# staghado/vit.cpp

Hardware: AMD Instinct MI355X
Metric: images/sec ViT-B/16 224^2 bs=256 per GPU (forward, synthetic, HBM-resident inputs) (higher is better)
Workload: dtype bf16

## Files before the change

vit.cpp_amd/csrc/engine.cpp:

```cpp
#include <hip/hip_runtime.h>
#include <stdio.h>
#include <stdlib.h>
#include <string.h>

#include <algorithm>
#include <map>
#include <memory>
#include <mutex>
#include <new>
#include <string>
#include <tuple>
#include <vector>

#include "kernels.h"
#include "model_file.h"

using namespace vitx;

#define HIP_TRY(expr)                                                                                      \
    do {                                                                                                   \
        hipError_t e__ = (expr);                                                                           \
        if (e__ != hipSuccess) { set_error("%s failed: %s (%s:%d)", #expr, hipGetErrorString(e__), __FILE__, __LINE__); return VITX_ERR_HIP; } \
    } while (0)

// ... 43 lines not shown
        void *pe_w = nullptr, *head_w = nullptr;
        QuantW head_q;
        std::vector<LayerW> layers;
        size_t weight_bytes = 0;
        ~WeightSet() {
            int cur = -1; (void)hipGetDevice(&cur);
            (void)hipSetDevice(device); for (void *p : allocs) (void)hipFree(p);
            if (cur >= 0 && cur != device) (void)hipSetDevice(cur);
        }
    };
    std::shared_ptr<WeightSet> wset;
    bool weights_shared = false;
    float *cls = nullptr, *pos = nullptr, *pe_b = nullptr, *norm_w = nullptr, *norm_b = nullptr, *head_b = nullptr;
    void *pe_w = nullptr, *head_w = nullptr;
    QuantW head_q;
    std::vector<LayerW> layers;
    bool quant_on_device = true;
    int q4_fused_rows = 0;
    size_t weight_bytes = 0;
    bool prec_attn = false;
    bool cls_tail = true;
    bool ln_fuse = true;
    unsigned ln_epoch = 0;
    unsigned ln_timeout = 20000;
    int ln_test = 0;
    int call_limit = 0;
    unsigned *ln_fb_host = nullptr;
    unsigned long long ln_fb_base = 0;
    int ln_fb_forwards = 0;
    bool ln_fuse_disabled = false;
    int ln_cool_left = 0, ln_cool_len = 256;
    struct Slice {
        int cap = 0;
        float *X = nullptr;
        void *U = nullptr;
        void *U2 = nullptr;
        unsigned long long *ln_sync = nullptr;
        unsigned *ln_todo = nullptr;
        int ln_blocks = 0;
        void *QKV = nullptr;
        long qkv_lo_off = 0;
        void *Hbuf = nullptr;
        float *Xc = nullptr;
        void *Z = nullptr;
        void *Wq[W_PER_LAYER] = {nullptr, nullptr, nullptr, nullptr};
        void *Wq_head = nullptr;
        float *logits = nullptr;
        hipStream_t stream = nullptr;
        hipEvent_t done = nullptr;
        Tuning tune;
    };
    int nslices = 1;
    std::vector<Slice> slices;
    hipEvent_t fork = nullptr;
    std::vector<hipStream_t> probed_streams;
    int stream_retries = 0;
    hipEvent_t probe_a = nullptr, probe_b = nullptr;
    float *img = nullptr;
    float *probs = nullptr;
    float *logits_all = nullptr;
// ... 173 lines not shown
    c->D = hp.hidden_size; c->L = hp.num_hidden_layers; c->H = hp.num_attention_heads; c->C = hp.num_classes; c->P = hp.patch_size; c->S = hp.img_size;
    c->Cin = m->in_chans; c->R = m->in_chans == 1 ? VITX_VITSTR_SEQ_LEN : 1;
    c->g = c->S / c->P; c->N = c->g * c->g + 1; c->Kpe = c->Cin * c->P * c->P; c->Kpe_pad = round_up(c->Kpe, 64);
    if (c->N < c->R) { set_error("vitx_ctx_create: a ViTSTR head reads %d tokens, this model has %d (img_size %d, patch_size %d)", c->R, c->N, c->S, c->P); return VITX_ERR_UNSUPPORTED; }
    c->tm = gemm_tile_m(); c->tn = gemm_tile_n();
    c->C_pad = round_up(c->C, c->tn);
    if (!attention_supports(c->N, c->D, c->H)) {
        set_error("vitx_ctx_create: attention needs a head_dim that is a multiple of 8 up to 128 (this model: %d) and at least one token (%d tokens, img_size %d, patch_size %d)", c->D / c->H, c->N, c->S, c->P);
        return VITX_ERR_UNSUPPORTED;
    }
    if (!layernorm_supports(c->D)) { set_error("vitx_ctx_create: hidden_size %d has no LayerNorm instantiation (64, 128, 192, 256, 320, 384, 448, 512, 576, 640, 768, 896, 1024, 1152, 1280, 1408, 1536, 1664, 2048)", c->D); return VITX_ERR_UNSUPPORTED; }
    c->tune = tuning_for_device(device);
    if (!c->tune) { set_error("vitx_ctx_create: kernel bring-up on device %d failed: %s", device, hipGetErrorString(hipGetLastError())); return VITX_ERR_HIP; }
    c->split_first = opt.split_first;
    c->prec_attn = dtype == VITX_F16 && c->D == c->H * 64 && !opt.f16_fast_attention;
    c->quant_on_device = !opt.quant_on_host;
    c->cls_tail = !opt.last_layer_all_rows && c->R == 1 && attention_cls_supports(c->N, c->D, c->H);
    c->q4_fused_rows = opt.q4_fused_rows;
    c->graphs_on = opt.graph != 0;
    if (opt.ln_test) {
        if ((opt.ln_test & (int32_t)0xffff0000) != (int32_t)VITX_LN_TEST_KEY) { set_error("vitx_ctx_create_ex: ln_test is a test-only switch (it needs its key: include/vitx.h)"); return VITX_ERR_ARG; }
        c->ln_test = opt.ln_test & 0xffff;
        if (c->ln_test & ~7) { set_error("vitx_ctx_create_ex: ln_test mode %d has bits outside 1 | 2 | 4", c->ln_test); return VITX_ERR_ARG; }
        if ((c->ln_test & 3) == 3) c->ln_timeout = 5000;
    }
    c->ln_fuse = !opt.no_ln_fusion && !opt.graph;
#ifdef VITX_LAB
    if (const char *e = getenv("VITX_SKIP")) c->skip = atoi(e);
    if (const char *e = getenv("VITX_SPLIT")) c->split_first = atoi(e);
#endif
    HIP_TRY(hipStreamCreateWithFlags(&c->stream, hipStreamNonBlocking));

    const int D = c->D, tn = c->tn;
    int rc;
    auto T = [&](const std::string &n) { return m->find(n); };
    static std::mutex wreg_mu;
    static std::map<std::tuple<uint64_t, int, int, int>, std::weak_ptr<vitx_ctx::WeightSet>> wreg;
    const auto wkey = std::make_tuple(m->uid, device, dtype, c->quant_on_device ? 1 : 0);
    std::unique_lock<std::mutex> wlock(wreg_mu);
    for (auto it = wreg.begin(); it != wreg.end();) it = it->second.expired() ? wreg.erase(it) : std::next(it);
    if (auto have = wreg[wkey].lock()) {
        c->wset = have; c->weights_shared = true;
    } else {
        c->wset = std::make_shared<vitx_ctx::WeightSet>();
        c->wset->device = device;
    }
    if (!c->weights_shared) {
// ... 35 lines not shown

    int ns = opt.streams > 0 ? opt.streams : 2;
    if (ns < 1) ns = 1;
    if (ns > 4) ns = 4;
    if (max_batch < 8 * ns) ns = 1;
    c->nslices = ns;
    c->slices.resize(ns);
    const size_t hcols = std::max<size_t>((size_t)4 * D, (size_t)c->Kpe_pad);
    {
        const size_t row_bytes = std::max<size_t>(hcols * 2, (size_t)3 * D * 2 * (c->prec_attn ? 2 : 1));
        const size_t rows = (size_t)0xf0000000u / row_bytes / 256 * 256;
        const long per_slice = (long)(rows / c->N);
        if (per_slice < 1) { set_error("vitx_ctx_create: a single image exceeds the kernels' 32-bit buffer window (%d tokens x %d)", c->N, D); return VITX_ERR_UNSUPPORTED; }
        c->call_limit = (int)std::min<long>((long)max_batch, per_slice);
    }
    for (int i = 0; i < ns; ++i) {
        vitx_ctx::Slice &sl = c->slices[i];
        sl.cap = std::min(max_batch, c->call_limit);
        const size_t Mpad = (size_t)round_up(sl.cap * c->N, c->tm), Bpad = (size_t)round_up(sl.cap * c->R, c->tm);
        if ((rc = c->dmalloc((void **)&sl.X, Mpad * D * 4, true))) return rc;
        if ((rc = c->dmalloc(&sl.U, Mpad * D * 2, true))) return rc;
        if ((rc = c->dmalloc(&sl.U2, Mpad * D * 2, true))) return rc;
        if (D % 256 == 0 && D / 256 <= 4) {
            if ((rc = c->dmalloc((void **)&sl.ln_sync, (Mpad / 256) * (size_t)(D / 256) * 256 * 2 * sizeof(unsigned long long), true))) return rc;
            if ((rc = c->dmalloc((void **)&sl.ln_todo, (Mpad / 256 + 1) * sizeof(unsigned), true))) return rc;
            sl.ln_blocks = (int)(Mpad / 256);
        }
        if ((rc = c->dmalloc(&sl.QKV, Mpad * 3 * D * 2 * (c->prec_attn ? 2 : 1), true))) return rc;
        sl.qkv_lo_off = c->prec_attn ? (long)(Mpad * 3 * D) : 0;
        if ((rc = c->dmalloc(&sl.Hbuf, Mpad * hcols * 2, true))) return rc;
        if ((rc = c->dmalloc(&sl.Z, Bpad * D * 2, true))) return rc;
        if (c->cls_tail && (rc = c->dmalloc((void **)&sl.Xc, Bpad * D * 4, true))) return rc;
        if ((rc = c->dmalloc((void **)&sl.logits, Bpad * c->C_pad * 4, true))) return rc;
        for (int k = 0; k < W_PER_LAYER; ++k) {
            size_t need = 0;
            for (const LayerW &w : c->layers) if (w.q[k].blocks) need = std::max(need, (size_t)w.q[k].n_pad * w.q[k].K * 2);
            if (need && (rc = c->dmalloc(&sl.Wq[k], need, false))) return rc;
        }
        if (c->head_q.blocks && (rc = c->dmalloc(&sl.Wq_head, (size_t)c->head_q.n_pad * c->head_q.K * 2, false))) return rc;
        sl.tune = *c->tune;
#ifdef VITX_LAB
        if (const char *e = getenv("VITX_SLICE_CU")) { if (ns > 1 && atoi(e) > 0) sl.tune.n_cu = atoi(e); }
#endif
        if (ns > 1 && i > 0) {
            int least = 0, greatest = 0;
            HIP_TRY(hipDeviceGetStreamPriorityRange(&least, &greatest));
            HIP_TRY(hipStreamCreateWithPriority(&sl.stream, hipStreamNonBlocking, greatest));
            HIP_TRY(hipEventCreateWithFlags(&sl.done, hipEventDisableTiming));
// ... 52 lines not shown
    auto fused_ok = [&](const QuantW &q, int rows) { return q.blocks && q.type == T_Q4_0 && rows <= c->q4_fused_rows && rows % 128 == 0 && q.n_pad % 128 == 0 && q.K % 64 == 0; };
    auto expand = [&](const QuantW *const *qs, void *const *dst, int count) -> int {
        bool done[W_PER_LAYER] = {false, false, false, false};
        for (int k = 0; k < count; ++k) {
            if (done[k] || !qs[k]) continue;
            DequantJob jobs[4]; int nj = 0; double bytes = 0;
            for (int m = k; m < count; ++m) {
                if (done[m] || !qs[m] || qs[m]->type != qs[k]->type) continue;
                jobs[nj++] = DequantJob{qs[m]->blocks, qs[m]->scales, dst[m], qs[m]->N, qs[m]->n_pad, qs[m]->K / 32};
                bytes += (double)qs[m]->N * qs[m]->K / 32 * type_block_bytes(qs[m]->type) + (double)qs[m]->n_pad * qs[m]->K * eb;
                done[m] = true;
            }
            ProfScope ps(c, st, PC_DEQUANT, 0, bytes);
            HIP_TRY(launch_dequant(dt, qs[k]->type, jobs, nj, st));
        }
        return VITX_OK;
    };
#ifdef VITX_LAB
    const int skip = c->skip;
#else
    constexpr int skip = 0;
#endif
    bool fuse = false;
    if (c->ln_fuse && sl.ln_sync) {
        GemmArgs probe{}; probe.M = M; probe.N = D; probe.N_pad = round_up(D, tn); probe.K = D; probe.lda = D; probe.ldw = D; probe.ldo = D;
        hipStreamCaptureStatus cs = hipStreamCaptureStatusNone;
        if (hipStreamIsCapturing(st, &cs) != hipSuccess) { (void)hipGetLastError(); cs = hipStreamCaptureStatusActive; }
        GemmArgs probe2 = probe; probe2.K = 4 * D; probe2.lda = 4 * D; probe2.ldw = 4 * D;
        fuse = cs == hipStreamCaptureStatusNone && gemm_ln_fusable(tn_, probe) && gemm_ln_fusable(tn_, probe2);
    }
    auto resid_gemm_ln = [&](int pc, const void *A, const void *W, const float *bias, int K, const QuantW *fq, const float *lw, const float *lb, void *ln_out, GemmLn *pend) -> int {
        int rc2;
        pend->todo = nullptr;
        if (fuse && lw && !fq) {
            GemmLn ln{};
            ln.w = lw; ln.b = lb; ln.x = sl.X; ln.out = ln_out; ln.eps = c->hp.eps; ln.sync = sl.ln_sync; ln.todo = sl.ln_todo; ln.fallbacks = sl.ln_todo + sl.ln_blocks;
            if (++c->ln_epoch == 0) c->ln_epoch = 1;
            ln.epoch = c->ln_epoch; ln.timeout = c->ln_timeout; ln.test = c->ln_test;
            if ((rc2 = gemm(c, tn_, st, pc, EPI_BIAS_RESID, A, W, bias, sl.X, nullptr, M, M, D, round_up(D, tn), K, K, K, D, 0, 4, nullptr, &ln, nullptr, 0, M_real))) return rc2;
            *pend = ln;
            return VITX_OK;
        }
        if ((rc2 = gemm(c, tn_, st, pc, EPI_BIAS_RESID, A, W, bias, sl.X, nullptr, M, M_real, D, round_up(D, tn), K, K, K, D, 0, 4, fq))) return rc2;
        if (lw) {
            ProfScope ps(c, st, PC_LAYERNORM, 0, (double)M_real * D * (4 + eb));
            if (!(skip & 2)) HIP_TRY(launch_layernorm(dt, sl.X, D, lw, lb, ln_out, D, M_real, D, c->hp.eps, st));
        }
        return VITX_OK;
    };
    GemmLn fix_u{}, fix_u2{};
    const bool tail = c->cls_tail && c->trace_ids.empty();
    const int Mc = round_up(n, tm);
    for (int il = 0; il < c->L; ++il) {
        const LayerW &w = c->layers[il];
        const bool tail_now = tail && il + 1 == c->L;
        const void *Wl[W_PER_LAYER] = {w.qkv_w, w.proj_w, w.fc1_w, w.fc2_w};
        const QuantW *Fl[W_PER_LAYER] = {nullptr, nullptr, nullptr, nullptr};
        {
            const QuantW *todo[W_PER_LAYER] = {nullptr, nullptr, nullptr, nullptr};
            bool any = false;
            for (int k = 0; k < W_PER_LAYER; ++k) {
// ... 88 lines not shown
        if (fused_ok(c->head_q, round_up(nR, tm))) head_f = &c->head_q;
        else { const QuantW *todo[1] = {&c->head_q}; void *dst[1] = {sl.Wq_head}; if ((rc = expand(todo, dst, 1))) return rc; head_w = sl.Wq_head; }
    }
    if ((rc = gemm(c, tn_, st, PC_GEMM_HEAD, EPI_BIAS_F32, sl.Z, head_w, c->head_b, lg, nullptr, round_up(nR, tm), nR, c->C, c->C_pad, D, D, D, ldl, 0, 4, head_f))) return rc;
    {
        ProfScope ps(c, st, PC_SOFTMAX, 0, (double)nR * c->C * 8);
        HIP_TRY(launch_softmax(dt, lg, (float *)d_probs, nR, c->C, ldl, st));
    }
    if (fuse && c->ln_fb_host) HIP_TRY(hipMemcpyAsync(c->ln_fb_host + (&sl - &c->slices[0]), sl.ln_todo + sl.ln_blocks, sizeof(unsigned), hipMemcpyDeviceToHost, st));
    return VITX_OK;
}

static double gemm_round_cost(long rows, int N, int K, int n_cu) {
    const long ntm = (rows + 255) / 256, ntn = (N + 255) / 256, tiles = ntm * ntn, rounds = tiles / n_cu, rem = tiles % n_cu;
    const double slots = K / 32.0, t_tile = slots * 0.98 + 3.5, t_half = slots * 0.6 + 3.0;
    if (rounds >= 1 && rem > 0 && rem <= n_cu * 6 / 10) {
        const long m_main = rounds * n_cu / ntn, half_tiles = ((ntm - m_main) * 2) * ntn;
        return rounds * t_tile + (double)((half_tiles + n_cu - 1) / n_cu) * t_half;
    }
    if (tiles < 128) return (double)(((rows + 127) / 128 * ntn + n_cu - 1) / n_cu) * t_half;
    return (double)((tiles + n_cu - 1) / n_cu) * t_tile;
}
static double gemm_round_cost_ln(long rows, int N, int K, int n_cu) {
    const long ntm = (rows + 255) / 256, ntn = N / 256;
    const int grid = gemm_ln_grid(n_cu, (int)(ntm * 256), N);
    const long most = ((ntm + 7) / 8) * ntn, wgx = grid / 8;
    return (double)((most + wgx - 1) / wgx) * (K / 32.0 * 0.98 + 3.5 + 2.0);
}
static void split_batch(const vitx_ctx *c, int n, int ns, int *m) {
    const int base = n / ns, extra = n % ns;
    for (int i = 0; i < ns; ++i) m[i] = base + (i < extra ? 1 : 0);
    if (c->split_first > 0 && ns == 2 && c->split_first < n) { m[0] = c->split_first; m[1] = n - c->split_first; return; }
    if (ns != 2) return;
    const int n_cu = c->tune->n_cu;
    const int D = c->D;
    const bool ln = c->ln_fuse && c->slices[0].ln_sync;
    if (ln) {
        const int ntn = D / 256, per_xcd = std::max(n_cu / 8, ntn) / ntn;
        const int s1 = (int)((long)8 * per_xcd * 256 / c->N);
        if (s1 >= n / 4 && s1 <= n / 2 && (long)s1 * c->N / 256 * ntn >= 128) { m[0] = s1; m[1] = n - s1; return; }
    }
    auto layer = [&](int imgs) {
        const long rows = (long)imgs * c->N;
        const bool fl = ln && ((rows + 255) / 256) * (D / 256) >= 128;
        return gemm_round_cost(rows, 3 * D, D, n_cu) + gemm_round_cost(rows, 4 * D, D, n_cu) +
               (fl ? gemm_round_cost_ln(rows, D, D, n_cu) + gemm_round_cost_ln(rows, D, 4 * D, n_cu) : gemm_round_cost(rows, D, D, n_cu) + gemm_round_cost(rows, D, 4 * D, n_cu));
    };
    double best = layer(m[0]) + layer(m[1]);
    for (int s1 = std::max(8, n / 4); s1 <= n / 2; ++s1) {
        const double cost = layer(s1) + layer(n - s1);
        if (cost < best * 0.97) { best = cost; m[0] = s1; m[1] = n - s1; }
    }
}

static int forward_graph(vitx_ctx *c, hipStream_t st, const void *d_imgs, int n, void *d_probs, void *d_logits, bool *done) {
    *done = false;
    for (auto &ge : c->graphs)
        if (ge.imgs == d_imgs && ge.n == n && ge.probs == d_probs && ge.logits == d_logits) {
            if (hipGraphLaunch(ge.exec, st) == hipSuccess) { *done = true; return VITX_OK; }
// ... 249 lines not shown
    g.M = M; g.M_real = M_real; g.N = N; g.N_pad = n_pad; g.K = K; g.lda = K; g.ldw = K; g.ldo = N; g.tpi = tpi;
    g.hilo_off = epi == EPI_BIAS_HILO ? (long)M * N : 0;
    hipError_t e = launch_gemm(t, dtype, epi, g, (hipStream_t)stream);
    if (e == hipErrorInvalidValue) { set_error("vitx_op_gemm: kernel %d cannot tile M %d N %d K %d", kernel, M, N, K); return VITX_ERR_UNSUPPORTED; }
    if (e != hipSuccess) { set_error("vitx_op_gemm: %s", hipGetErrorString(e)); return VITX_ERR_HIP; }
    return VITX_OK;
}
int vitx_op_gemm_ex(int dtype, int epi, int kernel, const void *a, const void *w, const void *bias, void *out, const void *pos, int M, int M_real, int N, int K, int tpi, void *stream) {
    return op_gemm_impl(dtype, epi, kernel, a, w, bias, out, pos, M, M_real, N, round_up(N, 256), K, tpi, stream);
}
int vitx_op_gemm(int dtype, int epi, const void *a, const void *w, const void *bias, void *out, int M, int N, int K, void *stream) {
    if (epi < 0 || epi > 3 || N % 64) { set_error("vitx_op_gemm: epi 0..3, N %% 64 == 0"); return VITX_ERR_ARG; }
    return op_gemm_impl(dtype, epi, 0, a, w, bias, out, nullptr, M, M, N, round_up(N, gemm_tile_n()), K, 0, stream);
}
int vitx_op_gemm_ln(int dtype, const void *a, const void *w, const void *bias, void *x, const void *ln_w, const void *ln_b, void *y, int M, int N, int K, float eps,
                    int test, int timeout_us, int *fallbacks, void *stream) {
    if (!a || !w || !bias || !x || !ln_w || !ln_b || !y || M <= 0 || timeout_us < 0) { set_error("vitx_op_gemm_ln: invalid argument"); return VITX_ERR_ARG; }
    const Tuning *t0 = tuning_for_device(-1);
    if (!t0) { set_error("vitx_op_gemm_ln: kernel bring-up failed"); return VITX_ERR_HIP; }
    GemmArgs g{};
    g.A = a; g.W = w; g.bias = (const float *)bias; g.out = x; g.M = M; g.M_real = M; g.N = N; g.N_pad = N; g.K = K; g.lda = K; g.ldw = K; g.ldo = N;
    if (!gemm_ln_fusable(*t0, g)) { set_error("vitx_op_gemm_ln: M %d N %d K %d does not take the LayerNorm-fusing kernel (M %% 256, N in {256,512,768,1024}, >= 128 tiles, K %% 128)", M, N, K); return VITX_ERR_UNSUPPORTED; }
    static unsigned epoch = 0x40000000u;
    const size_t nb = (size_t)M / 256, sync_bytes = nb * (N / 256) * 256 * 2 * sizeof(unsigned long long);
    unsigned long long *sync = nullptr; unsigned *todo = nullptr;
    HIP_TRY(hipMalloc((void **)&sync, sync_bytes));
    if (hipMalloc((void **)&todo, (nb + 1) * 4) != hipSuccess) { (void)hipFree(sync); return VITX_ERR_NOMEM; }
    int rc = VITX_OK;
    hipStream_t st = (hipStream_t)stream;
    GemmLn ln{};
    ln.w = (const float *)ln_w; ln.b = (const float *)ln_b; ln.out = y; ln.eps = eps; ln.sync = sync; ln.todo = todo; ln.fallbacks = todo + nb;
    ln.epoch = ++epoch; ln.timeout = (unsigned)timeout_us * 100u; ln.test = test;
    g.ln = &ln;
    hipError_t e = hipMemsetAsync(sync, 0, sync_bytes, st);
    if (e == hipSuccess) e = hipMemsetAsync(todo, 0, (nb + 1) * 4, st);
    if (e == hipSuccess) e = launch_gemm(*t0, dtype, EPI_BIAS_RESID, g, st);
    if (e == hipSuccess) e = launch_layernorm_fixup(dtype, (const float *)x, ln.w, ln.b, y, M, N, eps, todo, ln.epoch, st);
    if (e == hipSuccess) e = hipStreamSynchronize(st);
    unsigned fb = 0;
    if (e == hipSuccess) e = hipMemcpy(&fb, todo + nb, 4, hipMemcpyDeviceToHost);
    if (e != hipSuccess) { set_error("vitx_op_gemm_ln: %s", hipGetErrorString(e)); rc = VITX_ERR_HIP; }
    if (fallbacks) *fallbacks = (int)fb;
    (void)hipFree(sync); (void)hipFree(todo);
    return rc;
}
int vitx_op_dequant(int dtype, int qtype, const void *blocks, const void *scales, void *out, int N, int n_pad, int K, void *stream) {
    if (!blocks || !out || N <= 0 || n_pad < N || K <= 0 || K % 32 || (dtype != VITX_F16 && dtype != VITX_BF16)) { set_error("vitx_op_dequant: invalid argument"); return VITX_ERR_ARG; }
    DequantJob j{blocks, scales, out, N, n_pad, K / 32};
    hipError_t e = launch_dequant(dtype, qtype, &j, 1, (hipStream_t)stream);
    if (e != hipSuccess) { set_error("vitx_op_dequant: %s", hipGetErrorString(e)); return e == hipErrorInvalidValue ? VITX_ERR_ARG : VITX_ERR_HIP; }
    return VITX_OK;
}
int vitx_op_gemm_q4(int dtype, int epi, const void *a, const void *qs, const void *scales, const void *bias, void *out, int M, int M_real, int N, int K, void *stream) {
    if (!a || !qs || !scales || !bias || !out || epi < 0 || epi > EPI_BIAS_F32 || M_real <= 0 || M_real > M) { set_error("vitx_op_gemm_q4: invalid argument"); return VITX_ERR_ARG; }
    if (!tuning_for_device(-1)) { set_error("vitx_op_gemm_q4: kernel bring-up failed"); return VITX_ERR_HIP; }
    GemmArgs g{};
    g.A = a; g.W = qs; g.Wscale = (const uint16_t *)scales; g.bias = (const float *)bias; g.out = out;
    g.M = M; g.M_real = M_real; g.N = N; g.N_pad = round_up(N, 128); g.K = K; g.lda = K; g.ldw = K; g.ldo = N;
    hipError_t e = launch_gemm_q4(dtype, epi, g, (hipStream_t)stream);
    if (e == hipErrorInvalidValue) { set_error("vitx_op_gemm_q4: M %% 128, K %% 64 must be 0 (M %d N %d K %d)", M, N, K); return VITX_ERR_UNSUPPORTED; }
    if (e != hipSuccess) { set_error("vitx_op_gemm_q4: %s", hipGetErrorString(e)); return VITX_ERR_HIP; }
    return VITX_OK;
}
size_t vitx_ctx_weight_bytes(const vitx_ctx *c) { return c ? c->weight_bytes : 0; }
int vitx_ctx_shares_weights(const vitx_ctx *c) { return c && c->weights_shared ? 1 : 0; }
int vitx_ctx_stream_retries(const vitx_ctx *c) { return c ? c->stream_retries : -1; }
int vitx_ctx_ln_fusion_active(const vitx_ctx *c) { return c ? ((c->ln_fuse && !c->slices.empty() && c->slices[0].ln_sync && c->tune->n_xcd == 8) ? 1 : (c->ln_fuse_disabled ? -1 : 0)) : 0; }
long long vitx_ctx_ln_fallbacks(vitx_ctx *c) {
    if (!c) return -1;
    if (hipSetDevice(c->device) != hipSuccess || hipDeviceSynchronize() != hipSuccess) return -1;
    long long total = 0;
    for (auto &sl : c->slices) {
        if (!sl.ln_todo) continue;
        unsigned v = 0;
        if (hipMemcpy(&v, sl.ln_todo + sl.ln_blocks, sizeof v, hipMemcpyDeviceToHost) != hipSuccess) return -1;
        total += v;
    }
    return total;
}

int vitx_op_attention_ex(int dtype, int kernel, const void *qkv, void *out, int n_img, int N, int D, int H, void *stream) {
    if (!qkv || !out || n_img <= 0 || kernel < 0) return VITX_ERR_ARG;
    const Tuning *t0 = tuning_for_device(-1);
    if (!t0) { set_error("vitx_op_attention: kernel bring-up failed"); return VITX_ERR_HIP; }
    Tuning t = *t0;
#ifdef VITX_LAB
    t.attn_flags = kernel >> 4; kernel &= 15;
#endif
    if (kernel == ATTN_PERSIST) {
        if (N <= 192 || N > 224) { set_error("vitx_op_attention: the persistent kernel takes 193..224 tokens, not %d", N); return VITX_ERR_UNSUPPORTED; }
// ... 87 lines not shown
```

vit.cpp_amd/csrc/gemm_pp.hip:

```cpp
#include <stdio.h>
#include <stdlib.h>

#include <type_traits>

#include "device_common.h"
#include "kernels.h"
#include "epilogue16.h"

#ifndef PP_MAX_VGPR
#define PP_MAX_VGPR 128
#endif
#ifndef PP_AUX_QKV
#define PP_AUX_QKV 2
#endif
#ifndef PP_AUX_H
#define PP_AUX_H 2
#endif
#ifndef PP_AUX_A_LNF
#define PP_AUX_A_LNF 2
#endif
#ifndef PP_AUX_A
#define PP_AUX_A 0
#endif
#ifndef PP_RESID_DEPTH
// ... 4 lines not shown

namespace pp {
constexpr int BM = 256, BN = 256, BK = 64;
constexpr int HALF = 16384;
constexpr int LDS = 8 * HALF;
__host__ __device__ constexpr int off_a(int buf, int h) { return (buf * 2 + h) * HALF; }
__host__ __device__ constexpr int off_b(int buf, int h) { return (4 + buf * 2 + h) * HALF; }
constexpr int LDS_ALL = LDS + 8 * 4096;
constexpr int GROUP_M = 8;
constexpr int STAGE_OPS = 2;
constexpr int LEAD = 4;
}

template <int N> __device__ __forceinline__ void pp_wait_vmcnt() { asm volatile("s_waitcnt vmcnt(%0)" ::"n"(N) : "memory"); }
template <int N> __device__ __forceinline__ void pp_wait_vm_lgkm() { asm volatile("s_waitcnt vmcnt(%0) lgkmcnt(0)" ::"n"(N) : "memory"); }
__device__ __forceinline__ void pp_barrier() { asm volatile("s_barrier" ::: "memory"); }

template <int EPI> __host__ __device__ constexpr int pp_epi_stores() { return (EPI == EPI_BIAS || EPI == EPI_BIAS_GELU) ? 16 : 32; }

template <typename T>
__device__ __forceinline__ bool pp_epilogue_ln(const GemmArgs &g, const GemmLn &ln, f32x4 (&acc)[8][4], __amdgpu_buffer_rsrc_t ro, char *smem,
                                               int voff_in, int soff, int soff8, int tid_in, int m0, int n0, int ntn) {
    using namespace pp;
    typedef unsigned long long u64;
    int tid = tid_in, voff = voff_in;
    asm volatile("" : "+v"(tid), "+v"(voff));
    const int lane = tid & 63, wave = __builtin_amdgcn_readfirstlane(tid >> 6), wr = wave >> 2, wc = wave & 3;
    const int l15 = lane & 15, g4 = lane >> 4, lr = lane >> 3, lk = lane & 7;
    char *patch = smem + LDS + wave * 4096;
    char *sb = smem + off_a(1, 1);
    float *part = (float *)sb;
    float *cmean = (float *)(sb + 4096);
    float *stat = (float *)(sb + 5120);
    float *fin = (float *)(sb + 13312);
    int *fail = (int *)(sb + 15360);
    const int rd_off = lr * 128 + ((lk ^ (lr & 7)) * 16);
    const int mb = m0 / BM, ct = n0 / BN;
#define xv(b, j, t) acc[b][2 * (j) + (t)]
    {
        f32x4 br[2];
#pragma unroll
        for (int j = 0; j < 2; ++j) br[j] = *(const f32x4 *)(patch + j * 128 + lk * 16);
        pp_lds_fence();
        const int wr_row = l15 * 128, x16 = (l15 & 7) * 16;
        constexpr int RD = PP_RESID_DEPTH;
        u32x4 res[RD + 1][2];
        auto load_res = [&](int c, u32x4 (&dst)[2]) {
// ... 15 lines not shown
        for (int c = 0; c < 16; ++c) {
            const int b = c >> 1, j = c & 1;
            if (c + RD < 16) load_res(c + RD, res[(c + RD) % (RD + 1)]);
            f32x4 d[2];
#pragma unroll
            for (int t = 0; t < 2; ++t) d[t] = *(const f32x4 *)(patch + (c & 1) * 2048 + t * 1024 + rd_off);
            pp_lds_fence();
            if (c + 1 < 16) write_pass(c + 1);
#pragma unroll
            for (int t = 0; t < 2; ++t) {
                xv(b, j, t) = (d[t] + br[j]) + __builtin_bit_cast(f32x4, res[c % (RD + 1)][t]);
                asm volatile("" : "+v"(xv(b, j, t)));
            }
        }
    }
    f32x4 gw[2], gb[2];
#pragma unroll
    for (int j = 0; j < 2; ++j) { gw[j] = *(const f32x4 *)(ln.w + n0 + wc * 64 + j * 32 + lk * 4); gb[j] = *(const f32x4 *)(ln.b + n0 + wc * 64 + j * 32 + lk * 4); }
    auto store_x = [&]() {
#pragma unroll
        for (int c = 0; c < 16; ++c) {
            const int b = c >> 1, j = c & 1;
#pragma unroll
            for (int t = 0; t < 2; ++t) pp_store_b128(__builtin_bit_cast(u32x4, xv(b, j, t)), ro, voff + j * 128, soff + (b * 2 + t) * soff8);
        }
    };
    auto lds_barrier = [&]() { asm volatile("s_waitcnt lgkmcnt(0)\n\ts_barrier" ::: "memory"); };
    if (tid == 0) *fail = 0;
#pragma unroll
    for (int b = 0; b < 8; ++b)
#pragma unroll
        for (int t = 0; t < 2; ++t) {
            const float p = ln_sum8(ln_piece_sum(xv(b, 0, t)) + ln_piece_sum(xv(b, 1, t)));
            if (lk == 0) part[wc * 256 + wr * 128 + b * 16 + t * 8 + lr] = p;
            __builtin_amdgcn_sched_barrier(0);
        }
    lds_barrier();
    if (tid < 256) cmean[tid] = (((part[tid] + part[256 + tid]) + part[512 + tid]) + part[768 + tid]) * (1.0f / 256.0f);
    lds_barrier();
#pragma unroll
    for (int b = 0; b < 8; ++b)
#pragma unroll
        for (int t = 0; t < 2; ++t) {
            const float mc = cmean[wr * 128 + b * 16 + t * 8 + lr];
            const float q = ln_sum8(ln_piece_sq(xv(b, 0, t), mc) + ln_piece_sq(xv(b, 1, t), mc));
            if (lk == 0) part[wc * 256 + wr * 128 + b * 16 + t * 8 + lr] = q;
            __builtin_amdgcn_sched_barrier(0);
        }
    lds_barrier();
    const unsigned epoch = ln.epoch;
    const bool fake = (ln.test & 1) && ((mb * ntn + ct) % 5 == 0);
    {
        const int r = tid & 255;
        if (tid < 256) {
            const float m = cmean[r], q2 = ((part[r] + part[256 + r]) + part[512 + r]) + part[768 + r];
            stat[(ct * 256 + r) * 2] = m; stat[(ct * 256 + r) * 2 + 1] = q2;
            if (!(fake && (ln.test & 2))) {
                u64 *gp = ln.sync + ((size_t)(mb * ntn + ct) * 256 + r) * 2;
                __hip_atomic_store(gp, ((u64)epoch << 32) | __builtin_bit_cast(unsigned, m), __ATOMIC_RELAXED, __HIP_MEMORY_SCOPE_AGENT);
                __hip_atomic_store(gp + 1, ((u64)epoch << 32) | __builtin_bit_cast(unsigned, q2), __ATOMIC_RELAXED, __HIP_MEMORY_SCOPE_AGENT);
            }
        }
        for (int pi = tid >> 8; pi < ntn - 1; pi += 2) {
            const int c2 = pi < ct ? pi : pi + 1;
            const u64 *gp = ln.sync + ((size_t)(mb * ntn + c2) * 256 + r) * 2;
            const long long t_start = wall_clock64();
            bool ok = false;
            for (;;) {
                const u64 a = __hip_atomic_load(gp, __ATOMIC_RELAXED, __HIP_MEMORY_SCOPE_AGENT), b = __hip_atomic_load(gp + 1, __ATOMIC_RELAXED, __HIP_MEMORY_SCOPE_AGENT);
                if ((unsigned)(a >> 32) == epoch && (unsigned)(b >> 32) == epoch) {
                    stat[(c2 * 256 + r) * 2] = __builtin_bit_cast(float, (unsigned)a); stat[(c2 * 256 + r) * 2 + 1] = __builtin_bit_cast(float, (unsigned)b);
                    ok = true; break;
                }
                if (wall_clock64() - t_start > (long long)ln.timeout) break;
                __builtin_amdgcn_s_sleep(8);
            }
            if (!ok) *fail = 1;
        }
        if (fake && tid == 0) *fail = 1;
    }
    lds_barrier();
    if (*fail) {
        if (tid == 0) {
            __hip_atomic_store(ln.todo + mb, epoch, __ATOMIC_RELAXED, __HIP_MEMORY_SCOPE_AGENT);
            __hip_atomic_fetch_add(ln.fallbacks, 1u, __ATOMIC_RELAXED, __HIP_MEMORY_SCOPE_AGENT);
        }
        lds_barrier();
        store_x();
        asm volatile("s_waitcnt vmcnt(0)" ::: "memory");
        return false;
    }
    if (tid < 256) {
        float m_[LN_MAX_TILES], q_[LN_MAX_TILES];
#pragma unroll
        for (int c = 0; c < LN_MAX_TILES; ++c) { m_[c] = c < ntn ? stat[(c * 256 + tid) * 2] : 0.0f; q_[c] = c < ntn ? stat[(c * 256 + tid) * 2 + 1] : 0.0f; }
        float mean, rstd;
        ln_combine(m_, q_, ntn, g.N, ln.eps, mean, rstd);
        fin[tid * 2] = mean; fin[tid * 2 + 1] = rstd;
    }
    lds_barrier();
    {
        const __amdgpu_buffer_rsrc_t ru = __builtin_amdgcn_make_buffer_rsrc(ln.out, 0, (int)0xffffffffu, 0x00020000);
        const int uoff = voff >> 1, usoff = soff >> 1, usoff8 = soff8 >> 1;
        const bool odd = lk & 1;
        const int ucol = odd ? 64 + (lk - 1) * 8 : lk * 8;
#pragma unroll
        for (int b = 0; b < 8; ++b)
#pragma unroll
            for (int t = 0; t < 2; ++t) {
                const f32x2 mr = *(const f32x2 *)(fin + (wr * 128 + b * 16 + t * 8 + lr) * 2);
                unsigned pk[2][2];
#pragma unroll
                for (int j = 0; j < 2; ++j) {
                    float o[4];
#pragma unroll
                    for (int e = 0; e < 4; ++e) { float v = (xv(b, j, t)[e] - mr[0]) * mr[1]; v = v * gw[j][e]; o[e] = v + gb[j][e]; }
                    pk[j][0] = __builtin_bit_cast(unsigned, round_pair<T>(o[0], o[1])); pk[j][1] = __builtin_bit_cast(unsigned, round_pair<T>(o[2], o[3]));
                }
                const unsigned g0 = odd ? pk[0][0] : pk[1][0], g1 = odd ? pk[0][1] : pk[1][1];
                const unsigned r0 = (unsigned)__builtin_amdgcn_mov_dpp((int)g0, 0xB1, 0xf, 0xf, true), r1 = (unsigned)__builtin_amdgcn_mov_dpp((int)g1, 0xB1, 0xf, 0xf, true);
                const u32x4 d = odd ? u32x4{r0, r1, pk[1][0], pk[1][1]} : u32x4{pk[0][0], pk[0][1], r0, r1};
                __builtin_amdgcn_raw_buffer_store_b128(d, ru, uoff - lk * 8 + ucol, usoff + (b * 2 + t) * usoff8, 0);
                __builtin_amdgcn_sched_barrier(0); asm volatile("s_nop 1" ::: "memory"); __builtin_amdgcn_sched_barrier(0);
            }
    }
    store_x();
    lds_barrier();
    asm volatile("s_waitcnt vmcnt(32)" ::: "memory");
    return true;
#undef xv
}

template <typename T, int EPI, int FLAGS, bool LNF = false>
__global__ __launch_bounds__(512, 2) __attribute__((amdgpu_num_vgpr(PP_MAX_VGPR))) void gemm_pp_kernel(GemmArgs g, GemmLn ln) {
    using namespace pp;
    typedef typename Elem<T>::v8 v8;
    extern __shared__ __attribute__((aligned(16))) char smem[];

    const int tid = threadIdx.x, lane = tid & 63;
    const int wave = __builtin_amdgcn_readfirstlane(tid >> 6);
    const int wr = wave >> 2, wc = wave & 3;

    const int ntm = g.M / BM, ntn = g.N_pad / BN, ntiles = ntm * ntn;
    const int nblk = gridDim.x, bid = blockIdx.x;
    const int xcd = bid & 7;
    int my_tiles_, lid_base_;
    if constexpr (LNF) {
        const int qb = ntm >> 3, rb = ntm & 7;
        const int rows_x = qb + (xcd < rb ? 1 : 0), wgx = nblk >> 3, j = bid >> 3;
        lid_base_ = (xcd * qb + min(xcd, rb)) * ntn;
        my_tiles_ = j < rows_x * ntn ? (rows_x * ntn - j + wgx - 1) / wgx : 0;
    } else {
        const int q8 = ntiles >> 3, r8 = ntiles & 7;
        lid_base_ = (xcd < r8 ? xcd * (q8 + 1) : r8 * (q8 + 1) + (xcd - r8) * q8);
        my_tiles_ = (ntiles - bid + nblk - 1) / nblk;
    }
    const int my_tiles = my_tiles_, lid_base = lid_base_;
    const int group_m = g.group_m > 0 ? g.group_m : GROUP_M;
    auto tile_origin = [&](int round, int &m0, int &n0) {
        const int v = bid + round * nblk;
        const int lid = lid_base + (v >> 3);
        if constexpr (LNF) {
            const int mb = lid / ntn;
            m0 = mb * BM; n0 = (lid - mb * ntn) * BN;
        } else {
            const int per_group = group_m * ntn;
            const int grp = lid / per_group, within = lid - grp * per_group;
            const int gm = min(group_m, ntm - grp * group_m);
            const int tn = within / gm;
            m0 = (grp * group_m + (within - tn * gm)) * BM; n0 = tn * BN;
        }
    };
    if (my_tiles <= 0) return;
#ifdef VITX_LAB
    const long long lab_c0 = __builtin_readcyclecounter(), lab_r0 = __builtin_amdgcn_s_memrealtime();
#endif

    if constexpr (!LNF) {
        if (ln.todo) {
            bool any = false;
// ... 190 lines not shown
#undef PP_PHASE
}

bool gemm_pp_supports(const GemmArgs &a) {
    const size_t lim = 0xf0000000u;
    if ((size_t)a.M * a.lda * 2 > lim || (size_t)a.N_pad * a.ldw * 2 > lim || (size_t)(a.M + a.M / 64 + 2) * a.ldo * 4 + (size_t)(a.hilo_off > 0 ? a.hilo_off : 0) * 2 > lim) return false;
    return a.M % pp::BM == 0 && a.N_pad % pp::BN == 0 && a.K % (2 * pp::BK) == 0 && a.K >= 2 * pp::BK && a.N % 4 == 0 && a.ldo % 4 == 0;
}

template <typename T, int EPI, int FLAGS>
static hipError_t launch_pp_inst(const GemmArgs &a, int n_cu, hipStream_t stream, bool prepare) {
    if (prepare || FLAGS) {
        hipError_t e = hipFuncSetAttribute((const void *)gemm_pp_kernel<T, EPI, FLAGS>, hipFuncAttributeMaxDynamicSharedMemorySize, pp::LDS_ALL);
        if (prepare) return e;
    }
    const int ntiles = (a.M / pp::BM) * (a.N_pad / pp::BN);
    int cap = n_cu & ~7;
    if (cap <= 0) cap = 256;
    const int grid = ntiles < cap ? ntiles : cap;
    hipLaunchKernelGGL((gemm_pp_kernel<T, EPI, FLAGS>), dim3(grid), dim3(512), pp::LDS_ALL, stream, a, a.fix ? *a.fix : GemmLn{});
    return hipGetLastError();
}
int gemm_pp_ln_grid(int n_cu, int M, int N) {
    const int ntm = M / pp::BM, ntn = N / pp::BN;
    int per_xcd = (n_cu > 0 ? n_cu : 256) / 8;
    if (per_xcd < ntn) per_xcd = ntn;
    const int cap = per_xcd / ntn * ntn;
    const int most = ((ntm + 7) / 8) * ntn;
    const int rounds = (most + cap - 1) / cap;
    int wgx = ((most + rounds - 1) / rounds + ntn - 1) / ntn * ntn;
    if (wgx > cap) wgx = cap;
    return 8 * wgx;
}
template <typename T>
static hipError_t launch_pp_ln(const GemmArgs &a, int n_cu, hipStream_t stream, bool prepare) {
    if (prepare) return hipFuncSetAttribute((const void *)gemm_pp_kernel<T, EPI_BIAS_RESID, 0, true>, hipFuncAttributeMaxDynamicSharedMemorySize, pp::LDS_ALL);
    const GemmLn &ln = *a.ln;
    if (!ln.w || !ln.b || !ln.out || !ln.sync || !ln.todo || !ln.fallbacks || !ln.epoch || a.N != a.N_pad || a.N != a.ldo || a.N / pp::BN > LN_MAX_TILES) return hipErrorInvalidValue;
    hipLaunchKernelGGL((gemm_pp_kernel<T, EPI_BIAS_RESID, 0, true>), dim3(gemm_pp_ln_grid(n_cu, a.M, a.N)), dim3(512), pp::LDS_ALL, stream, a, ln);
    return hipGetLastError();
}
template <typename T>
static hipError_t launch_pp_t(int epi, const GemmArgs &a, int n_cu, hipStream_t stream, int flags, bool prepare) {
#ifdef VITX_LAB
    if (flags) {
        if (epi != EPI_BIAS) return hipErrorInvalidValue;
        switch (flags) {
        case 1: return launch_pp_inst<T, EPI_BIAS, 1>(a, n_cu, stream, prepare);
        case 4: return launch_pp_inst<T, EPI_BIAS, 4>(a, n_cu, stream, prepare);
        case 8: return launch_pp_inst<T, EPI_BIAS, 8>(a, n_cu, stream, prepare);
        case 12: return launch_pp_inst<T, EPI_BIAS, 12>(a, n_cu, stream, prepare);
        case 16: return launch_pp_inst<T, EPI_BIAS, 16>(a, n_cu, stream, prepare);
        case 32: return launch_pp_inst<T, EPI_BIAS, 32>(a, n_cu, stream, prepare);
        case 512: return launch_pp_inst<T, EPI_BIAS, 512>(a, n_cu, stream, prepare);
        case 2048: return launch_pp_inst<T, EPI_BIAS, 2048>(a, n_cu, stream, prepare);
        case 4096: return launch_pp_inst<T, EPI_BIAS, 4096>(a, n_cu, stream, prepare);
        default: return hipErrorInvalidValue;
        }
    }
#else
    if (flags) return hipErrorInvalidValue;
// ... 23 lines not shown
```

vit.cpp_amd/csrc/kernels.h:

```cpp
#pragma once
#include <hip/hip_runtime.h>
#include <stdint.h>

namespace vitx {

enum { DT_F16 = 0, DT_BF16 = 1 };

enum {
    EPI_BIAS = 0,
    EPI_BIAS_GELU = 1,
    EPI_BIAS_RESID = 2,
    EPI_BIAS_F32 = 3,
    EPI_PATCH = 4,
    EPI_BIAS_HILO = 5
};
constexpr float kHiLoScale = 2048.0f, kHiLoInv = 1.0f / 2048.0f;

struct GemmArgs {
    const void *A; const void *W; const float *bias; void *out; const float *pos;
    int M;
    int M_real;
    int N;
    int N_pad;
    int K;
    int lda, ldw, ldo;
    int tpi;
    long hilo_off;
    int dbg;
    const uint16_t *Wscale;
    int group_m;
    const struct GemmLn *ln;
    const struct GemmLn *fix;
};

struct GemmLn {
    const float *w, *b;
    const float *x;
    void *out;
    float eps;
    unsigned long long *sync;
    unsigned *todo;
    unsigned *fallbacks;
    unsigned epoch;
    unsigned timeout;
    int test;
};

enum { QT_Q4_0 = 2, QT_Q4_1 = 3, QT_Q5_0 = 6, QT_Q5_1 = 7, QT_Q8_0 = 8 };
struct DequantJob { const void *src; const void *scales; void *dst; int N, n_pad, nbk; };
hipError_t launch_dequant(int dtype, int qtype, const DequantJob *jobs, int njobs, hipStream_t stream);
hipError_t launch_gemm_q4(int dtype, int epi, const GemmArgs &a, hipStream_t stream);
bool gemm_q4_supports(const GemmArgs &a);

enum { ATTN_AUTO = 0, ATTN_SINGLE = 1, ATTN_FLOW = 3, ATTN_PERSIST = 4, ATTN_STREAM = 5 };
struct Tuning {
    int device = 0;
    int n_cu = 256;
    int n_xcd = 8;
    int gemm_cfg = -1;
    int skinny_tiles = 128;
    int gemm_split = 0;
    int gemm_balance = 1;
    int group_m = 0;
    int pp_flags = 0;
    int gemm_dbg = 0;
    int attn_kernel = ATTN_AUTO;
    int attn_flags = 0;
// ... 41 lines not shown
```

Before: 26990.

## Replace spin-wait LayerNorm stat exchange with last-arriver ticket finalization in fused GEMM

The fused GEMM+LayerNorm epilogue used to have every column tile of a row block publish its partial stats, then spin-wait with a timeout for its sibling tiles. Each tile then normalized its own columns. Now each tile publishes packed stats, writes its residual output, and takes an atomic ticket. Only the last tile to arrive for a row block reads all the stats and normalizes the full row block, reloading the other tiles' fp32 output from memory. This removes the co-residency requirement and the spinning, so the grid no longer has to be XCD-aligned and can be balanced across all tiles. The cost is that one workgroup per row block does the extra normalization work serially, re-reading data from global memory.

```diff
diff --git a/vit.cpp_amd/csrc/engine.cpp b/vit.cpp_amd/csrc/engine.cpp
--- a/vit.cpp_amd/csrc/engine.cpp
+++ b/vit.cpp_amd/csrc/engine.cpp
@@ -89,7 +89,6 @@
     bool cls_tail = true;
     bool ln_fuse = true;
     unsigned ln_epoch = 0;
-    unsigned ln_timeout = 20000;
     int ln_test = 0;
     int call_limit = 0;
     unsigned *ln_fb_host = nullptr;
@@ -102,7 +101,7 @@
         float *X = nullptr;
         void *U = nullptr;
         void *U2 = nullptr;
-        unsigned long long *ln_sync = nullptr;
+        float *ln_stat = nullptr;
         unsigned *ln_todo = nullptr;
         int ln_blocks = 0;
         void *QKV = nullptr;
@@ -322,7 +321,6 @@
         if ((opt.ln_test & (int32_t)0xffff0000) != (int32_t)VITX_LN_TEST_KEY) { set_error("vitx_ctx_create_ex: ln_test is a test-only switch (it needs its key: include/vitx.h)"); return VITX_ERR_ARG; }
         c->ln_test = opt.ln_test & 0xffff;
         if (c->ln_test & ~7) { set_error("vitx_ctx_create_ex: ln_test mode %d has bits outside 1 | 2 | 4", c->ln_test); return VITX_ERR_ARG; }
-        if ((c->ln_test & 3) == 3) c->ln_timeout = 5000;
     }
     c->ln_fuse = !opt.no_ln_fusion && !opt.graph;
 #ifdef VITX_LAB
@@ -404,8 +402,8 @@
         if ((rc = c->dmalloc(&sl.U, Mpad * D * 2, true))) return rc;
         if ((rc = c->dmalloc(&sl.U2, Mpad * D * 2, true))) return rc;
         if (D % 256 == 0 && D / 256 <= 4) {
-            if ((rc = c->dmalloc((void **)&sl.ln_sync, (Mpad / 256) * (size_t)(D / 256) * 256 * 2 * sizeof(unsigned long long), true))) return rc;
-            if ((rc = c->dmalloc((void **)&sl.ln_todo, (Mpad / 256 + 1) * sizeof(unsigned), true))) return rc;
+            if ((rc = c->dmalloc((void **)&sl.ln_stat, (Mpad / 256) * (size_t)(D / 256) * 256 * 2 * sizeof(float), true))) return rc;
+            if ((rc = c->dmalloc((void **)&sl.ln_todo, (2 * (Mpad / 256) + 1) * sizeof(unsigned), true))) return rc;
             sl.ln_blocks = (int)(Mpad / 256);
         }
         if ((rc = c->dmalloc(&sl.QKV, Mpad * 3 * D * 2 * (c->prec_attn ? 2 : 1), true))) return rc;
@@ -504,7 +502,7 @@
     constexpr int skip = 0;
 #endif
     bool fuse = false;
-    if (c->ln_fuse && sl.ln_sync) {
+    if (c->ln_fuse && sl.ln_stat) {
         GemmArgs probe{}; probe.M = M; probe.N = D; probe.N_pad = round_up(D, tn); probe.K = D; probe.lda = D; probe.ldw = D; probe.ldo = D;
         hipStreamCaptureStatus cs = hipStreamCaptureStatusNone;
         if (hipStreamIsCapturing(st, &cs) != hipSuccess) { (void)hipGetLastError(); cs = hipStreamCaptureStatusActive; }
@@ -516,9 +514,9 @@
         pend->todo = nullptr;
         if (fuse && lw && !fq) {
             GemmLn ln{};
-            ln.w = lw; ln.b = lb; ln.x = sl.X; ln.out = ln_out; ln.eps = c->hp.eps; ln.sync = sl.ln_sync; ln.todo = sl.ln_todo; ln.fallbacks = sl.ln_todo + sl.ln_blocks;
+            ln.w = lw; ln.b = lb; ln.x = sl.X; ln.out = ln_out; ln.eps = c->hp.eps; ln.stat = sl.ln_stat; ln.arrive = sl.ln_todo + sl.ln_blocks + 1; ln.todo = sl.ln_todo; ln.fallbacks = sl.ln_todo + sl.ln_blocks;
             if (++c->ln_epoch == 0) c->ln_epoch = 1;
-            ln.epoch = c->ln_epoch; ln.timeout = c->ln_timeout; ln.test = c->ln_test;
+            ln.epoch = c->ln_epoch; ln.test = c->ln_test;
             if ((rc2 = gemm(c, tn_, st, pc, EPI_BIAS_RESID, A, W, bias, sl.X, nullptr, M, M, D, round_up(D, tn), K, K, K, D, 0, 4, nullptr, &ln, nullptr, 0, M_real))) return rc2;
             *pend = ln;
             return VITX_OK;
@@ -653,10 +651,9 @@
     return (double)((tiles + n_cu - 1) / n_cu) * t_tile;
 }
 static double gemm_round_cost_ln(long rows, int N, int K, int n_cu) {
-    const long ntm = (rows + 255) / 256, ntn = N / 256;
+    const long ntm = (rows + 255) / 256, ntn = N / 256, tiles = ntm * ntn;
     const int grid = gemm_ln_grid(n_cu, (int)(ntm * 256), N);
-    const long most = ((ntm + 7) / 8) * ntn, wgx = grid / 8;
-    return (double)((most + wgx - 1) / wgx) * (K / 32.0 * 0.98 + 3.5 + 2.0);
+    return (double)((tiles + grid - 1) / grid) * (K / 32.0 * 0.98 + 3.5 + 2.0);
 }
 static void split_batch(const vitx_ctx *c, int n, int ns, int *m) {
     const int base = n / ns, extra = n % ns;
@@ -665,7 +662,7 @@
     if (ns != 2) return;
     const int n_cu = c->tune->n_cu;
     const int D = c->D;
-    const bool ln = c->ln_fuse && c->slices[0].ln_sync;
+    const bool ln = c->ln_fuse && c->slices[0].ln_stat;
     if (ln) {
         const int ntn = D / 256, per_xcd = std::max(n_cu / 8, ntn) / ntn;
         const int s1 = (int)((long)8 * per_xcd * 256 / c->N);
@@ -961,18 +958,18 @@
     g.A = a; g.W = w; g.bias = (const float *)bias; g.out = x; g.M = M; g.M_real = M; g.N = N; g.N_pad = N; g.K = K; g.lda = K; g.ldw = K; g.ldo = N;
     if (!gemm_ln_fusable(*t0, g)) { set_error("vitx_op_gemm_ln: M %d N %d K %d does not take the LayerNorm-fusing kernel (M %% 256, N in {256,512,768,1024}, >= 128 tiles, K %% 128)", M, N, K); return VITX_ERR_UNSUPPORTED; }
     static unsigned epoch = 0x40000000u;
-    const size_t nb = (size_t)M / 256, sync_bytes = nb * (N / 256) * 256 * 2 * sizeof(unsigned long long);
-    unsigned long long *sync = nullptr; unsigned *todo = nullptr;
+    const size_t nb = (size_t)M / 256, sync_bytes = nb * (N / 256) * 256 * 2 * sizeof(float);
+    float *sync = nullptr; unsigned *todo = nullptr;
     HIP_TRY(hipMalloc((void **)&sync, sync_bytes));
-    if (hipMalloc((void **)&todo, (nb + 1) * 4) != hipSuccess) { (void)hipFree(sync); return VITX_ERR_NOMEM; }
+    if (hipMalloc((void **)&todo, (2 * nb + 1) * 4) != hipSuccess) { (void)hipFree(sync); return VITX_ERR_NOMEM; }
     int rc = VITX_OK;
     hipStream_t st = (hipStream_t)stream;
     GemmLn ln{};
-    ln.w = (const float *)ln_w; ln.b = (const float *)ln_b; ln.out = y; ln.eps = eps; ln.sync = sync; ln.todo = todo; ln.fallbacks = todo + nb;
-    ln.epoch = ++epoch; ln.timeout = (unsigned)timeout_us * 100u; ln.test = test;
+    ln.w = (const float *)ln_w; ln.b = (const float *)ln_b; ln.out = y; ln.eps = eps; ln.stat = sync; ln.arrive = todo + nb + 1; ln.todo = todo; ln.fallbacks = todo + nb;
+    ln.epoch = ++epoch; ln.test = test;
     g.ln = &ln;
     hipError_t e = hipMemsetAsync(sync, 0, sync_bytes, st);
-    if (e == hipSuccess) e = hipMemsetAsync(todo, 0, (nb + 1) * 4, st);
+    if (e == hipSuccess) e = hipMemsetAsync(todo, 0, (2 * nb + 1) * 4, st);
     if (e == hipSuccess) e = launch_gemm(*t0, dtype, EPI_BIAS_RESID, g, st);
     if (e == hipSuccess) e = launch_layernorm_fixup(dtype, (const float *)x, ln.w, ln.b, y, M, N, eps, todo, ln.epoch, st);
     if (e == hipSuccess) e = hipStreamSynchronize(st);
@@ -1004,7 +1001,7 @@
 size_t vitx_ctx_weight_bytes(const vitx_ctx *c) { return c ? c->weight_bytes : 0; }
 int vitx_ctx_shares_weights(const vitx_ctx *c) { return c && c->weights_shared ? 1 : 0; }
 int vitx_ctx_stream_retries(const vitx_ctx *c) { return c ? c->stream_retries : -1; }
-int vitx_ctx_ln_fusion_active(const vitx_ctx *c) { return c ? ((c->ln_fuse && !c->slices.empty() && c->slices[0].ln_sync && c->tune->n_xcd == 8) ? 1 : (c->ln_fuse_disabled ? -1 : 0)) : 0; }
+int vitx_ctx_ln_fusion_active(const vitx_ctx *c) { return c ? ((c->ln_fuse && !c->slices.empty() && c->slices[0].ln_stat && c->tune->n_xcd == 8) ? 1 : (c->ln_fuse_disabled ? -1 : 0)) : 0; }
 long long vitx_ctx_ln_fallbacks(vitx_ctx *c) {
     if (!c) return -1;
     if (hipSetDevice(c->device) != hipSuccess || hipDeviceSynchronize() != hipSuccess) return -1;
diff --git a/vit.cpp_amd/csrc/gemm_pp.hip b/vit.cpp_amd/csrc/gemm_pp.hip
--- a/vit.cpp_amd/csrc/gemm_pp.hip
+++ b/vit.cpp_amd/csrc/gemm_pp.hip
@@ -50,7 +50,6 @@
 __device__ __forceinline__ bool pp_epilogue_ln(const GemmArgs &g, const GemmLn &ln, f32x4 (&acc)[8][4], __amdgpu_buffer_rsrc_t ro, char *smem,
                                                int voff_in, int soff, int soff8, int tid_in, int m0, int n0, int ntn) {
     using namespace pp;
-    typedef unsigned long long u64;
     int tid = tid_in, voff = voff_in;
     asm volatile("" : "+v"(tid), "+v"(voff));
     const int lane = tid & 63, wave = __builtin_amdgcn_readfirstlane(tid >> 6), wr = wave >> 2, wc = wave & 3;
@@ -112,7 +111,7 @@
         for (int c = 0; c < 16; ++c) {
             const int b = c >> 1, j = c & 1;
 #pragma unroll
-            for (int t = 0; t < 2; ++t) pp_store_b128(__builtin_bit_cast(u32x4, xv(b, j, t)), ro, voff + j * 128, soff + (b * 2 + t) * soff8);
+            for (int t = 0; t < 2; ++t) pp_store_b128<16>(__builtin_bit_cast(u32x4, xv(b, j, t)), ro, voff + j * 128, soff + (b * 2 + t) * soff8);
         }
     };
     auto lds_barrier = [&]() { asm volatile("s_waitcnt lgkmcnt(0)\n\ts_barrier" ::: "memory"); };
@@ -140,50 +139,46 @@
     lds_barrier();
     const unsigned epoch = ln.epoch;
     const bool fake = (ln.test & 1) && ((mb * ntn + ct) % 5 == 0);
-    {
-        const int r = tid & 255;
-        if (tid < 256) {
-            const float m = cmean[r], q2 = ((part[r] + part[256 + r]) + part[512 + r]) + part[768 + r];
-            stat[(ct * 256 + r) * 2] = m; stat[(ct * 256 + r) * 2 + 1] = q2;
-            if (!(fake && (ln.test & 2))) {
-                u64 *gp = ln.sync + ((size_t)(mb * ntn + ct) * 256 + r) * 2;
-                __hip_atomic_store(gp, ((u64)epoch << 32) | __builtin_bit_cast(unsigned, m), __ATOMIC_RELAXED, __HIP_MEMORY_SCOPE_AGENT);
-                __hip_atomic_store(gp + 1, ((u64)epoch << 32) | __builtin_bit_cast(unsigned, q2), __ATOMIC_RELAXED, __HIP_MEMORY_SCOPE_AGENT);
-            }
-        }
-        for (int pi = tid >> 8; pi < ntn - 1; pi += 2) {
-            const int c2 = pi < ct ? pi : pi + 1;
-            const u64 *gp = ln.sync + ((size_t)(mb * ntn + c2) * 256 + r) * 2;
-            const long long t_start = wall_clock64();
-            bool ok = false;
-            for (;;) {
-                const u64 a = __hip_atomic_load(gp, __ATOMIC_RELAXED, __HIP_MEMORY_SCOPE_AGENT), b = __hip_atomic_load(gp + 1, __ATOMIC_RELAXED, __HIP_MEMORY_SCOPE_AGENT);
-                if ((unsigned)(a >> 32) == epoch && (unsigned)(b >> 32) == epoch) {
-                    stat[(c2 * 256 + r) * 2] = __builtin_bit_cast(float, (unsigned)a); stat[(c2 * 256 + r) * 2 + 1] = __builtin_bit_cast(float, (unsigned)b);
-                    ok = true; break;
-                }
-                if (wall_clock64() - t_start > (long long)ln.timeout) break;
-                __builtin_amdgcn_s_sleep(8);
-            }
-            if (!ok) *fail = 1;
-        }
-        if (fake && tid == 0) *fail = 1;
-    }
-    lds_barrier();
-    if (*fail) {
-        if (tid == 0) {
-            __hip_atomic_store(ln.todo + mb, epoch, __ATOMIC_RELAXED, __HIP_MEMORY_SCOPE_AGENT);
-            __hip_atomic_fetch_add(ln.fallbacks, 1u, __ATOMIC_RELAXED, __HIP_MEMORY_SCOPE_AGENT);
-        }
+    if (tid < 256) {
+        const int r = tid;
+        const float m = cmean[r], q2 = ((part[r] + part[256 + r]) + part[512 + r]) + part[768 + r];
+        stat[(ct * 256 + r) * 2] = m; stat[(ct * 256 + r) * 2 + 1] = q2;
+        if (!(fake && (ln.test & 2)))
+            __hip_atomic_store((unsigned long long *)ln.stat + ((size_t)(mb * ntn + ct) * 256 + r), ((unsigned long long)__builtin_bit_cast(unsigned, q2) << 32) | __builtin_bit_cast(unsigned, m),
+                               __ATOMIC_RELAXED, __HIP_MEMORY_SCOPE_AGENT);
+    }
+    if (fake && tid == 0) {
+        __hip_atomic_store(ln.todo + mb, epoch, __ATOMIC_RELAXED, __HIP_MEMORY_SCOPE_AGENT);
+        __hip_atomic_fetch_add(ln.fallbacks, 1u, __ATOMIC_RELAXED, __HIP_MEMORY_SCOPE_AGENT);
+    }
+    store_x();
+    asm volatile("s_waitcnt vmcnt(0)" ::: "memory");
+    lds_barrier();
+    if (tid == 0) {
+        const unsigned ticket = __hip_atomic_fetch_add(ln.arrive + mb, 1u, __ATOMIC_RELAXED, __HIP_MEMORY_SCOPE_AGENT);
+        int last = ticket == (unsigned)(ntn - 1);
+        if (last) {
+            __hip_atomic_store(ln.arrive + mb, 0u, __ATOMIC_RELAXED, __HIP_MEMORY_SCOPE_AGENT);
+            if (__hip_atomic_load(ln.todo + mb, __ATOMIC_RELAXED, __HIP_MEMORY_SCOPE_AGENT) == epoch) last = 0;
+        }
+        *fail = last;
+    }
+    lds_barrier();
+    if (!*fail) {
         lds_barrier();
-        store_x();
-        asm volatile("s_waitcnt vmcnt(0)" ::: "memory");
         return false;
     }
     if (tid < 256) {
         float m_[LN_MAX_TILES], q_[LN_MAX_TILES];
 #pragma unroll
-        for (int c = 0; c < LN_MAX_TILES; ++c) { m_[c] = c < ntn ? stat[(c * 256 + tid) * 2] : 0.0f; q_[c] = c < ntn ? stat[(c * 256 + tid) * 2 + 1] : 0.0f; }
+        for (int c = 0; c < LN_MAX_TILES; ++c) {
+            m_[c] = 0.0f; q_[c] = 0.0f;
+            if (c < ntn && c == ct) { m_[c] = stat[(c * 256 + tid) * 2]; q_[c] = stat[(c * 256 + tid) * 2 + 1]; }
+            else if (c < ntn) {
+                const unsigned long long v = __hip_atomic_load((const unsigned long long *)ln.stat + ((size_t)(mb * ntn + c) * 256 + tid), __ATOMIC_RELAXED, __HIP_MEMORY_SCOPE_AGENT);
+                m_[c] = __builtin_bit_cast(float, (unsigned)v); q_[c] = __builtin_bit_cast(float, (unsigned)(v >> 32));
+            }
+        }
         float mean, rstd;
         ln_combine(m_, q_, ntn, g.N, ln.eps, mean, rstd);
         fin[tid * 2] = mean; fin[tid * 2 + 1] = rstd;
@@ -214,10 +209,31 @@
                 __builtin_amdgcn_sched_barrier(0); asm volatile("s_nop 1" ::: "memory"); __builtin_amdgcn_sched_barrier(0);
             }
     }
-    store_x();
-    lds_barrier();
-    asm volatile("s_waitcnt vmcnt(32)" ::: "memory");
-    return true;
+    {
+        T *yb = (T *)ln.out + (size_t)m0 * g.ldo;
+        for (int c = 0; c < ntn; ++c) {
+            if (c == ct) continue;
+            const int col = c * BN + lane * 4;
+            const f32x4 ww = *(const f32x4 *)(ln.w + col), bb = *(const f32x4 *)(ln.b + col);
+            for (int r0 = wave; r0 < BM; r0 += 64) {
+                f32x4 xr[8];
+#pragma unroll
+                for (int i = 0; i < 8; ++i) xr[i] = __builtin_bit_cast(f32x4, __builtin_amdgcn_raw_buffer_load_b128(ro, (int)((unsigned)((m0 + r0 + i * 8) * g.ldo + col) * 4u), 0, 16));
+#pragma unroll
+                for (int i = 0; i < 8; ++i) {
+                    const f32x2 mr = *(const f32x2 *)(fin + (r0 + i * 8) * 2);
+                    float o[4];
+#pragma unroll
+                    for (int e = 0; e < 4; ++e) { float v = (xr[i][e] - mr[0]) * mr[1]; v = v * ww[e]; o[e] = v + bb[e]; }
+                    const typename Pair<T>::v2 lo = round_pair<T>(o[0], o[1]), hi = round_pair<T>(o[2], o[3]);
+                    *(typename Elem<T>::v4 *)(yb + (size_t)(r0 + i * 8) * g.ldo + col) = typename Elem<T>::v4{lo[0], lo[1], hi[0], hi[1]};
+                }
+            }
+        }
+    }
+    lds_barrier();
+    asm volatile("s_waitcnt vmcnt(0)" ::: "memory");
+    return false;
 #undef xv
 }
 
@@ -234,18 +250,9 @@
     const int ntm = g.M / BM, ntn = g.N_pad / BN, ntiles = ntm * ntn;
     const int nblk = gridDim.x, bid = blockIdx.x;
     const int xcd = bid & 7;
-    int my_tiles_, lid_base_;
-    if constexpr (LNF) {
-        const int qb = ntm >> 3, rb = ntm & 7;
-        const int rows_x = qb + (xcd < rb ? 1 : 0), wgx = nblk >> 3, j = bid >> 3;
-        lid_base_ = (xcd * qb + min(xcd, rb)) * ntn;
-        my_tiles_ = j < rows_x * ntn ? (rows_x * ntn - j + wgx - 1) / wgx : 0;
-    } else {
-        const int q8 = ntiles >> 3, r8 = ntiles & 7;
-        lid_base_ = (xcd < r8 ? xcd * (q8 + 1) : r8 * (q8 + 1) + (xcd - r8) * q8);
-        my_tiles_ = (ntiles - bid + nblk - 1) / nblk;
-    }
-    const int my_tiles = my_tiles_, lid_base = lid_base_;
+    const int q8 = ntiles >> 3, r8 = ntiles & 7;
+    const int lid_base = (xcd < r8 ? xcd * (q8 + 1) : r8 * (q8 + 1) + (xcd - r8) * q8);
+    const int my_tiles = (ntiles - bid + nblk - 1) / nblk;
     const int group_m = g.group_m > 0 ? g.group_m : GROUP_M;
     auto tile_origin = [&](int round, int &m0, int &n0) {
         const int v = bid + round * nblk;
@@ -482,21 +489,19 @@
     return hipGetLastError();
 }
 int gemm_pp_ln_grid(int n_cu, int M, int N) {
-    const int ntm = M / pp::BM, ntn = N / pp::BN;
-    int per_xcd = (n_cu > 0 ? n_cu : 256) / 8;
-    if (per_xcd < ntn) per_xcd = ntn;
-    const int cap = per_xcd / ntn * ntn;
-    const int most = ((ntm + 7) / 8) * ntn;
-    const int rounds = (most + cap - 1) / cap;
-    int wgx = ((most + rounds - 1) / rounds + ntn - 1) / ntn * ntn;
-    if (wgx > cap) wgx = cap;
-    return 8 * wgx;
+    int cap = (n_cu > 0 ? n_cu : 256) & ~7;
+    if (cap <= 0) cap = 256;
+    const long ntiles = (long)(M / pp::BM) * (N / pp::BN);
+    if (ntiles <= cap) return (int)((ntiles + 7) & ~7L);
+    const long rounds = (ntiles + cap - 1) / cap;
+    const long g = ((ntiles + rounds - 1) / rounds + 7) & ~7L;
+    return (int)(g < cap ? g : cap);
 }
 template <typename T>
 static hipError_t launch_pp_ln(const GemmArgs &a, int n_cu, hipStream_t stream, bool prepare) {
     if (prepare) return hipFuncSetAttribute((const void *)gemm_pp_kernel<T, EPI_BIAS_RESID, 0, true>, hipFuncAttributeMaxDynamicSharedMemorySize, pp::LDS_ALL);
     const GemmLn &ln = *a.ln;
-    if (!ln.w || !ln.b || !ln.out || !ln.sync || !ln.todo || !ln.fallbacks || !ln.epoch || a.N != a.N_pad || a.N != a.ldo || a.N / pp::BN > LN_MAX_TILES) return hipErrorInvalidValue;
+    if (!ln.w || !ln.b || !ln.out || !ln.stat || !ln.arrive || !ln.todo || !ln.fallbacks || !ln.epoch || a.N != a.N_pad || a.N != a.ldo || a.N / pp::BN > LN_MAX_TILES) return hipErrorInvalidValue;
     hipLaunchKernelGGL((gemm_pp_kernel<T, EPI_BIAS_RESID, 0, true>), dim3(gemm_pp_ln_grid(n_cu, a.M, a.N)), dim3(512), pp::LDS_ALL, stream, a, ln);
     return hipGetLastError();
 }
diff --git a/vit.cpp_amd/csrc/kernels.h b/vit.cpp_amd/csrc/kernels.h
--- a/vit.cpp_amd/csrc/kernels.h
+++ b/vit.cpp_amd/csrc/kernels.h
@@ -38,11 +38,11 @@
     const float *x;
     void *out;
     float eps;
-    unsigned long long *sync;
+    float *stat;
+    unsigned *arrive;
     unsigned *todo;
     unsigned *fallbacks;
     unsigned epoch;
-    unsigned timeout;
     int test;
 };
 
```

Result: no change. 26720 (median of 6 runs) (-1.0%).
